# sidd-bme/macaque-3d-pose-estimation

Hardware: AMD Instinct MI355X
Metric: individuals×frames/sec 3D pose (8-view ViTPose-h + triangulate), 1/2/4/8 GPU (higher is better)
Workload: dtype bf16

## Files before the change

### include/mq_hip.h

```cpp
#ifndef MQ_HIP_H
#define MQ_HIP_H

#include <stdint.h>

#ifdef __cplusplus
extern "C" {
#endif

#define MQ_ABI_VERSION 8

typedef struct mq_ctx mq_ctx;
typedef struct mq_vitpose mq_vitpose;

int mq_abi_version(void);
const char* mq_last_error(void);

#define MQ_TUNE_GEMM_FORCE_SMALL 2
#define MQ_TUNE_OPTIM_PCG_ITERS 4
#define MQ_TUNE_GEMM_PINGPONG 12
#define MQ_TUNE_OPTIM_PRECOND_LDS 18
#define MQ_TUNE_GEMM_TILE64 19
#define MQ_TUNE_QKV_HEAD_MAJOR 20
#define MQ_TUNE_OPTIM_STOP 21
#define MQ_TUNE_VIT_RESID_F32 23
#define MQ_TUNE_ATTN_KRING 24
#define MQ_TUNE_OPTIM_TRF_CHUNK 22
#define MQ_TUNE_OPTIM_TRF_FB 25
#define MQ_TUNE_GEMM_W4 27
int mq_set_tuning(int key, int value);
int mq_get_tuning(int key);
int mq_create(int device, mq_ctx** out);
int mq_destroy(mq_ctx* ctx);


int mq_vitpose_create(mq_ctx* ctx, int embed_dims, int num_layers, int num_heads, int ffn_dims, int n_joints,
                      mq_vitpose** out);
int mq_vitpose_destroy(mq_vitpose* model);

int mq_vitpose_set_param(mq_vitpose* model, const char* name, const float* data, int64_t numel, int on_device);

int mq_vitpose_finalize(mq_vitpose* model);

int mq_vitpose_set_graph(mq_vitpose* model, int enable);

int mq_vitpose_timing(mq_vitpose* model, int enable);
int mq_vitpose_timing_result(mq_vitpose* model, double* avg_ms, int* count, int64_t* flops_per_launch);

int mq_crop_udp(mq_ctx* ctx, const uint8_t* frames, int64_t frame_stride, int height, int width,
                const float* boxes, const int32_t* box_frame, int n, float* crops, float* center, float* scale,
                void* stream);

// ... 197 lines not shown
```

### macaque-3d-pose-estimation_amd/csrc/api.cpp

```cpp
#include <hip/hip_runtime.h>

#include <algorithm>
#include <cmath>
#include <cstdio>
#include <cstring>
#include <map>
#include <string>
#include <vector>

#include "bundle.hpp"
#include "cmc.hpp"
#include "geometry.hpp"
#include "overlay.hpp"
#include "detector.hpp"
#include "idcls.hpp"
#include "kernels.hpp"
#include "mq_hip.h"

namespace {

thread_local std::string g_err;
int g_qkv_head_major = 1;
int g_vit_resid_f32 = 0;
int g_tuning_gen = 0;
// ... 127 lines not shown
      break;
    case MQ_TUNE_VIT_RESID_F32:
      g_vit_resid_f32 = value != 0;
      break;
    case MQ_TUNE_ATTN_KRING:
      mq::g_attn_kring = value != 0;
      break;
    case MQ_TUNE_OPTIM_STOP:
      if (value < 0 || value > 7) return fail("mq_set_tuning: optim stop rule must be in [0, 7]", -2);
      mq::g_optim_stop = value;
      break;
    case MQ_TUNE_OPTIM_TRF_CHUNK:
      if (value < 1 || value > 64) return fail("mq_set_tuning: lsmr chunk must be in [1, 64]", -2);
      mq::g_optim_trf_chunk = value;
      break;
    case MQ_TUNE_OPTIM_TRF_FB:
      if (value < 1 || value > 4) return fail("mq_set_tuning: frames per workgroup must be in [1, 4]", -2);
      mq::g_optim_trf_fb = value;
      break;
    case MQ_TUNE_GEMM_W4:
      if (value < 0 || value > 2) return fail("mq_set_tuning: GEMM_W4 must be 0, 1 or 2", -2);
      mq::g_gemm_w4 = value;
      break;
    default:
      return fail("mq_set_tuning: unknown key", -2);
  }
  ++g_tuning_gen;
  return 0;
}

int mq_get_tuning(int key) {
  switch (key) {
    case MQ_TUNE_GEMM_FORCE_SMALL: return mq::g_gemm_force_small ? 1 : 0;
    case MQ_TUNE_GEMM_PINGPONG: return mq::g_gemm_pingpong;
    case MQ_TUNE_OPTIM_PCG_ITERS: return mq::g_optim_pcg_iters;
    case MQ_TUNE_OPTIM_PRECOND_LDS: return mq::g_optim_precond_lds;
    case MQ_TUNE_GEMM_TILE64: return mq::g_gemm_tile64;
    case MQ_TUNE_QKV_HEAD_MAJOR: return g_qkv_head_major;
    case MQ_TUNE_VIT_RESID_F32: return g_vit_resid_f32;
    case MQ_TUNE_ATTN_KRING: return mq::g_attn_kring;
    case MQ_TUNE_OPTIM_STOP: return mq::g_optim_stop;
    case MQ_TUNE_OPTIM_TRF_CHUNK: return mq::g_optim_trf_chunk;
    case MQ_TUNE_OPTIM_TRF_FB: return mq::g_optim_trf_fb;
    case MQ_TUNE_GEMM_W4: return mq::g_gemm_w4;
    default: return fail("mq_get_tuning: unknown key", -2);
  }
}

const char* mq_last_error(void) { return g_err.c_str(); }

int mq_create(int device, mq_ctx** out) {
  if (!out) return fail("mq_create: null out");
  int n = 0;
  HIP_TRY(hipGetDeviceCount(&n));
  if (device < 0 || device >= n) return fail("mq_create: bad device index");
  HIP_TRY(hipSetDevice(device));
  mq_ctx* c = new mq_ctx();
  c->device = device;
  *out = c;
  return 0;
}

int mq_destroy(mq_ctx* ctx) {
  if (!ctx) return 0;
  (void)hipSetDevice(ctx->device);
  ctx->scratch.release();
  ctx->decode_work.release();
// ... 352 lines not shown
      K_TRY(gemm_plain(g, s));
  }
  if (m->L > 0 && !rf32)
    K_TRY(mq::add_layernorm_f32_bf16(m->X, P1, P2, false, m->lnf_g, m->lnf_b, m->Hn, rows, D, 1e-6f, s));
  else
    K_TRY(mq::layernorm_f32_bf16(m->X, m->lnf_g, m->lnf_b, m->Hn, rows, D, 1e-6f, s));
  unsigned short* cols1 = m->G;
  g = mq::GemmArgs{m->Hn, m->w_dc1, cols1, nullptr, nullptr, rows, 16 * dc, D, D, D, 16 * dc, 0};
  K_TRY(gemm_plain(g, s));
  K_TRY(mq::deconv_col2im_bn_relu(cols1, m->bn1_scale, m->bn1_shift, m->Y1, F, m->gh, m->gw, dc, s));
  const int rows2 = F * 4 * T;
  if (m->dc2_subpixel) {
    g = mq::GemmArgs{m->Y1, m->w_dc2, m->Y2, m->bn2_shift4, nullptr, rows2, 4 * dc, 4 * dc, dc, 4 * dc, dc, 0};
    g.conv_h = 2 * m->gh;
    g.conv_w = 2 * m->gw;
    g.conv_c = dc;
    K_TRY(mq::deconv_subpixel_bf16(g, mq::EPI_RELU_BF16, s));
  } else {
    g = mq::GemmArgs{m->Y1, m->w_dc2, m->cols2, nullptr, nullptr, rows2, 16 * dc, dc, dc, dc, 16 * dc, 0};
    K_TRY(mq::gemm_bf16(g, mq::EPI_BF16, s));
    K_TRY(mq::deconv_col2im_bn_relu(m->cols2, m->bn2_scale, m->bn2_shift, m->Y2, F, 2 * m->gh, 2 * m->gw, dc, s));
  }
  const int rows3 = F * 16 * T;
  float* hm_dst = flip ? m->hm_all : heatmaps;
  g = mq::GemmArgs{m->Y2, m->w_fin, hm_dst, m->b_fin, nullptr, rows3, m->J, dc, dc, dc, m->J, 16 * T};
  K_TRY(mq::gemm_bf16(g, mq::EPI_NCHW_F32, s));
  if (flip) K_TRY(mq::flip_average(m->hm_all, heatmaps, n, m->J, 4 * m->gh, 4 * m->gw, m->flip_idx, s));
  return 0;
}

int mq_vitpose_forward(mq_vitpose* m, const float* crops, int n, int flip_test, float* heatmaps, void* stream) {
  if (!m || !crops || !heatmaps) return fail("mq_vitpose_forward: null argument");
  if (!m->finalized) return fail("mq_vitpose_forward: model not finalized", -2);
  if (n <= 0) return 0;
  HIP_TRY(hipSetDevice(m->ctx->device));
  hipStream_t s = (hipStream_t)stream;
  const int F = flip_test ? 2 * n : n;
  int rc = ensure_workspace(m, F);
  if (rc) return rc;
  if (!m->use_graph || m->timing) return launch_forward(m, crops, n, flip_test, heatmaps, s);
  if (!m->cap_stream) {
    HIP_TRY(hipStreamCreateWithFlags(&m->cap_stream, hipStreamNonBlocking));
    HIP_TRY(hipEventCreateWithFlags(&m->ev_in, hipEventDisableTiming));
    HIP_TRY(hipEventCreateWithFlags(&m->ev_out, hipEventDisableTiming));
  }
  hipStream_t cs = m->cap_stream;
// ... 458 lines not shown
  K_TRY(mq::omnidir_undistort(cams, C, pts, out, n, (hipStream_t)stream));
  return 0;
}

int mq_omnidir_project(mq_ctx* ctx, const double* cams, int C, const double* p3d, int n, double* out, void* stream) {
  int rc = check_geo(ctx, cams, C, n);
  if (rc) return rc;
  K_TRY(mq::omnidir_project(cams, C, p3d, out, n, (hipStream_t)stream));
  return 0;
}

int mq_camera_undistort(mq_ctx* ctx, const double* cams, int C, const double* pts, int n, double* out, void* stream) {
  return mq_omnidir_undistort(ctx, cams, C, pts, n, out, stream);
}

int mq_camera_project(mq_ctx* ctx, const double* cams, int C, const double* p3d, int n, double* out, void* stream) {
  return mq_omnidir_project(ctx, cams, C, p3d, n, out, stream);
}

int mq_triangulate_dlt(mq_ctx* ctx, const double* cams, int C, const double* pts, int n, int undistort, double* out,
                       void* stream) {
  int rc = check_geo(ctx, cams, C, n);
  if (rc) return rc;
  if (undistort && n > 0) {
    if (ctx->dlt_ws.ensure((size_t)C * n * 2 * sizeof(double))) return fail("DLT workspace alloc failed", -5);
    K_TRY(mq::omnidir_undistort(cams, C, pts, ctx->dlt_ws.as<double>(), n, (hipStream_t)stream));
    K_TRY(mq::triangulate_dlt(cams, C, ctx->dlt_ws.as<double>(), n, 0, out, (hipStream_t)stream));
    return 0;
  }
  K_TRY(mq::triangulate_dlt(cams, C, pts, n, undistort, out, (hipStream_t)stream));
  return 0;
}

int mq_reproj_error(mq_ctx* ctx, const double* cams, int C, const double* p3d, const double* p2d, int n, int mean,
                    double* out, void* stream) {
  int rc = check_geo(ctx, cams, C, n);
  if (rc) return rc;
  K_TRY(mq::reprojection_error(cams, C, p3d, p2d, n, mean, out, (hipStream_t)stream));
  return 0;
}

int mq_triangulate_ransac(mq_ctx* ctx, const double* cams, int C, const double* pts, int n, int min_cams,
                          double threshold, double* p3d, uint8_t* picked, double* p2d, double* err, void* stream) {
  int rc = check_geo(ctx, cams, C, n);
  if (rc) return rc;
  K_TRY(mq::triangulate_ransac(cams, C, pts, n, min_cams, threshold, p3d, picked, p2d, err, (hipStream_t)stream));
  return 0;
// ... 467 lines not shown
```

### macaque-3d-pose-estimation_amd/csrc/geometry.hip

```cpp
#include "common.hpp"
#include "camera.hpp"
#include "geometry.hpp"
#include "dlt_dev.hpp"

namespace mq {

template <int MAXC>
__device__ __forceinline__ void dlt_point(const double* cams, int C, const double* ux, const double* uy,
                                          unsigned use, double out[3]) {
  double a[4][2 * MAXC];
#pragma unroll
  for (int c = 0; c < MAXC; ++c) {
    const bool on = (c < C) && ((use >> c) & 1u);
    if (on) {
      const CamParams& cp = cam_at(cams, c);
      const double P0[4] = {cp.R[0], cp.R[1], cp.R[2], cp.t[0]};
      const double P1[4] = {cp.R[3], cp.R[4], cp.R[5], cp.t[1]};
      const double P2[4] = {cp.R[6], cp.R[7], cp.R[8], cp.t[2]};
#pragma unroll
      for (int k = 0; k < 4; ++k) {
        a[k][2 * c] = ux[c] * P2[k] - P0[k];
        a[k][2 * c + 1] = uy[c] * P2[k] - P1[k];
      }
    } else {
// ... 193 lines not shown
  unsigned use = 0;
  int cnt = 0;
#pragma unroll
  for (int c = 0; c < MAXC; ++c) {
    ux[c] = 0;
    uy[c] = 0;
    if (c < C) {
      const double u = pts[2 * ((size_t)c * N + n)], v = pts[2 * ((size_t)c * N + n) + 1];
      double x = u, y = v;
      if (undistort) cam_undistort(cam_at(cams, c), u, v, x, y);
      ux[c] = x;
      uy[c] = y;
      if (!(x != x)) {
        use |= 1u << c;
        ++cnt;
      }
    }
  }
  double r[3] = {NAN, NAN, NAN};
  if (cnt >= 2) dlt_point<MAXC>(cams, C, ux, uy, use, r);
  out[3 * n] = r[0];
  out[3 * n + 1] = r[1];
  out[3 * n + 2] = r[2];
}

__global__ void reproj_kernel(const double* __restrict__ cams, int C, const double* __restrict__ p3d,
                              const double* __restrict__ p2d, int N, int mean, double* __restrict__ out) {
  const int n = blockIdx.x * blockDim.x + threadIdx.x;
  if (n >= N) return;
  const double X = p3d[3 * n], Y = p3d[3 * n + 1], Z = p3d[3 * n + 2];
  double sum = 0.0, cnt = 0.0;
  for (int c = 0; c < C; ++c) {
    double u, v;
    cam_project(cam_at(cams, c), X, Y, Z, u, v);
    const size_t o = 2 * ((size_t)c * N + n);
    const double ex = p2d[o] - u, ey = p2d[o + 1] - v;
    if (!mean) {
      out[o] = ex;
      out[o + 1] = ey;
    } else {
      const double nr = sqrt(ex * ex + ey * ey);
      if (!(nr != nr)) {
        sum = sum + nr;
        cnt = cnt + 1.0;
      }
    }
// ... 316 lines not shown
    double* o = out + ((((size_t)a * F + i) * V.C + c) * V.J + j) * 3;
    o[0] = r[0];
    o[1] = r[1];
    o[2] = r[2];
  }
}

int omnidir_undistort(const double* cams, int C, const double* pts, double* out, int N, hipStream_t s) {
  const int tot = C * N;
  if (tot <= 0) return 0;
  hipLaunchKernelGGL(undistort_kernel, dim3((tot + 255) / 256), dim3(256), 0, s, cams, C, pts, out, N);
  return hipGetLastError() == hipSuccess ? 0 : -1;
}

int omnidir_project(const double* cams, int C, const double* p3d, double* out, int N, hipStream_t s) {
  const int tot = C * N;
  if (tot <= 0) return 0;
  hipLaunchKernelGGL(project_kernel, dim3((tot + 255) / 256), dim3(256), 0, s, cams, C, p3d, out, N);
  return hipGetLastError() == hipSuccess ? 0 : -1;
}

int triangulate_dlt(const double* cams, int C, const double* pts, int N, int undistort, double* out, hipStream_t s) {
  if (N <= 0) return 0;
  if (C <= 8)
    hipLaunchKernelGGL(triangulate_kernel<8>, dim3((N + 63) / 64), dim3(64), 0, s, cams, C, pts, N, undistort, out);
  else if (C <= 16)
    hipLaunchKernelGGL(triangulate_kernel<16>, dim3((N + 63) / 64), dim3(64), 0, s, cams, C, pts, N, undistort, out);
  else
    return -2;
  return hipGetLastError() == hipSuccess ? 0 : -1;
}

int reprojection_error(const double* cams, int C, const double* p3d, const double* p2d, int N, int mean, double* out,
                       hipStream_t s) {
  if (N <= 0) return 0;
  hipLaunchKernelGGL(reproj_kernel, dim3((N + 127) / 128), dim3(128), 0, s, cams, C, p3d, p2d, N, mean, out);
  return hipGetLastError() == hipSuccess ? 0 : -1;
}

int triangulate_ransac(const double* cams, int C, const double* pts, int N, int min_cams, double threshold,
                       double* p3d, uint8_t* picked, double* p2d, double* err, hipStream_t s) {
  if (N <= 0) return 0;
  if (C <= 8)
    hipLaunchKernelGGL(ransac_kernel<8>, dim3(N), dim3(64), 0, s, cams, C, pts, N, min_cams, threshold, p3d, picked,
                       p2d, err);
  else if (C <= 16)
// ... 71 lines not shown
```

### macaque-3d-pose-estimation_amd/csrc/geometry.hpp

```cpp
#pragma once
#include <hip/hip_runtime.h>
#include <stdint.h>

namespace mq {
int omnidir_undistort(const double* cams, int C, const double* pts, double* out, int N, hipStream_t s);
int omnidir_project(const double* cams, int C, const double* p3d, double* out, int N, hipStream_t s);
int triangulate_dlt(const double* cams, int C, const double* pts, int N, int undistort, double* out, hipStream_t s);
int reprojection_error(const double* cams, int C, const double* p3d, const double* p2d, int N, int mean, double* out,
                       hipStream_t s);
int triangulate_ransac(const double* cams, int C, const double* pts, int N, int min_cams, double threshold,
                       double* p3d, uint8_t* picked, double* p2d, double* err, hipStream_t s);
int triangulate_pinv(const double* cams, int C, const double* und, const uint8_t* use, int N, double* out,
                     hipStream_t s);
int geometry_affinity(const double* cams, int C, const double* pts, const int32_t* cam_of_det, int B, int M, int J,
                      double thr_kp, double* rays, double* dist, double* out, hipStream_t s);
int viterbi_filter(const double* kp, int A, int F, int C, int J, double score_thr, int n_back, double thres_dist,
                   void* scratch, double* out, hipStream_t s);
size_t viterbi_scratch_bytes(int A, int F, int C, int J, int n_back);
int match_svt(const double* S, const int32_t* n_det, const int32_t* cam_of_det, int B, int Nmax, double alpha,
              double lambda, double mu, double tol, int max_iter, int pselect, void* ws, uint8_t* match,
              double* x_out, int32_t* iters, hipStream_t s);
size_t match_svt_workspace_bytes(int B, int Nmax);
int tracklet_traces(const double* cams, int C, const int32_t* row_start, const int32_t* row_tid,
                    const double* row_kp, int R, int F, int J, const int32_t* trk, int K, const int32_t* cells,
                    int N, double thr_kp, double* p3d, double* median, double* mean, hipStream_t s);
int tracklet_id_votes(int C, const int32_t* row_start, const int32_t* row_tid, const int32_t* row_cls,
                      const double* row_score, int R, int F, const int32_t* trk, int K, const int32_t* cells, int N,
                      double conf_thr, int n_class, int32_t* votes, hipStream_t s);
}
```

### macaque-3d-pose-estimation_amd/csrc/imgproc.hip

```cpp
#include "common.hpp"
#include "kernels.hpp"

namespace mq {

struct BoxWarp {
  float c0, c1, s0, s1;
  double M[6];
};

__device__ __forceinline__ BoxWarp box_warp(const float* bb, int out_w, int out_h) {
  BoxWarp w;
  const float x1 = bb[0], y1 = bb[1], x2 = bb[2], y2 = bb[3];
  const float sw = (x2 - x1) * 1.25f, sh = (y2 - y1) * 1.25f;
  w.c0 = (x2 + x1) * 0.5f;
  w.c1 = (y2 + y1) * 0.5f;
  const float ar = 0.75f;
  if (sw > sh * ar) {
    w.s0 = sw;
    w.s1 = sw / ar;
  } else {
    w.s0 = sh * ar;
    w.s1 = sh;
  }
  const double in0 = (double)(w.c0 * 2.0f), in1 = (double)(w.c1 * 2.0f);
// ... 54 lines not shown
#pragma unroll
  for (int tap = 0; tap < 4; ++tap) {
    const int yy = sy + (tap >> 1), xx = sx + (tap & 1);
    const int wgt = tap == 0 ? w00 : tap == 1 ? w01 : tap == 2 ? w10 : w11;
    if (yy >= 0 && yy < H && xx >= 0 && xx < W) {
      const uint8_t* p = img + ((int64_t)yy * W + xx) * 3;
      acc[0] += p[0] * wgt;
      acc[1] += p[1] * wgt;
      acc[2] += p[2] * wgt;
    }
  }
  const float mean[3] = {123.675f, 116.28f, 103.53f};
  const float stdv[3] = {58.395f, 57.12f, 57.375f};
  const int64_t plane = (int64_t)out_h * out_w;
  float* out = crops + (int64_t)n * 3 * plane + (int64_t)y * out_w + x;
#pragma unroll
  for (int c = 0; c < 3; ++c) {
    int v = (acc[2 - c] + 16384) >> 15;
    v = v < 0 ? 0 : (v > 255 ? 255 : v);
    out[c * plane] = ((float)v - mean[c]) / stdv[c];
  }
}

int crop_udp(const uint8_t* frames, int64_t frame_stride, int img_h, int img_w, const float* boxes,
             const int32_t* box_frame, int n, float* crops, float* center, float* scale, hipStream_t s) {
  if (n <= 0) return 0;
  const int out_w = 192, out_h = 256;
  hipLaunchKernelGGL(crop_udp_kernel, dim3(out_h, n), dim3(256), 0, s, frames, frame_stride, img_h, img_w, boxes,
                     box_frame, crops, center, scale, out_w, out_h);
  return hipGetLastError() == hipSuccess ? 0 : -1;
}

__global__ void flip_average_kernel(const float* __restrict__ hm, float* __restrict__ avg, int N, int K, int HH,
                                    int WW, const int32_t* __restrict__ fi) {
  const int64_t plane = (int64_t)HH * WW;
  const int64_t total = (int64_t)N * K * plane;
  for (int64_t i = blockIdx.x * (int64_t)blockDim.x + threadIdx.x; i < total; i += (int64_t)gridDim.x * blockDim.x) {
    const int x = (int)(i % WW);
    const int y = (int)((i / WW) % HH);
    const int k = (int)((i / plane) % K);
    const int n = (int)(i / (plane * K));
    const float a = hm[i];
    const float b = hm[(((int64_t)(n + N) * K + fi[k]) * HH + y) * WW + (WW - 1 - x)];
    avg[i] = (a + b) * 0.5f;
  }
}

int flip_average(const float* hm_all, float* avg, int n, int joints, int h, int w, const int32_t* flip_idx,
                 hipStream_t s) {
  const int64_t total = (int64_t)n * joints * h * w;
  int blocks = (int)((total + 255) / 256);
  if (blocks > 8192) blocks = 8192;
  hipLaunchKernelGGL(flip_average_kernel, dim3(blocks), dim3(256), 0, s, hm_all, avg, n, joints, h, w, flip_idx);
  return hipGetLastError() == hipSuccess ? 0 : -1;
}

__constant__ float kGauss11[11] = {
    0.00881222914904356f, 0.027143577113747597f, 0.06511405855417252f, 0.12164907157421112f,
    0.17699836194515228f, 0.2005654126405716f,   0.17699836194515228f, 0.12164907157421112f,
    0.06511405855417252f, 0.027143577113747597f, 0.00881222914904356f};

__global__ __launch_bounds__(256) void decode_blur_kernel(const float* __restrict__ avg, int K, int HH, int WW,
                                                          float* __restrict__ work, int32_t* __restrict__ argmax,
                                                          float* __restrict__ score) {
  extern __shared__ __attribute__((aligned(16))) float sm[];
  const int nk = blockIdx.x;
  const int plane = HH * WW;
  const int PR = HH + 10;
  float* hmap = sm;
  float* rows = sm + plane;
  __shared__ float red_v[256];
  __shared__ int red_i[256];
  const float* src = avg + (int64_t)nk * plane;
  float bv = -INFINITY;
  int bi = 0x7fffffff;
  for (int i = threadIdx.x; i < plane; i += blockDim.x) {
// ... 50 lines not shown
  }
  __syncthreads();
  float lmax = -INFINITY;
  for (int i = threadIdx.x; i < plane; i += blockDim.x) {
    const int y = i / WW, x = i % WW;
    float acc = kGauss11[0] * rows[y * WW + x];
    for (int t = 1; t < 11; ++t) acc = acc + kGauss11[t] * rows[(y + t) * WW + x];
    hmap[i] = acc;
    lmax = fmaxf(lmax, acc);
  }
  __syncthreads();
  red_v[threadIdx.x] = lmax;
  __syncthreads();
  for (int o = 128; o > 0; o >>= 1) {
    if (threadIdx.x < o) red_v[threadIdx.x] = fmaxf(red_v[threadIdx.x], red_v[threadIdx.x + o]);
    __syncthreads();
  }
  const float ratio = origin_max / red_v[0];
  float* dst = work + (int64_t)nk * plane;
  for (int i = threadIdx.x; i < plane; i += blockDim.x) {
    float v = hmap[i] * ratio;
    v = fminf(fmaxf(v, 0.001f), 50.0f);
    dst[i] = logf(v);
  }
}

__device__ __forceinline__ float padded_at(const float* work_inst, int K, int HH, int WW, long idx) {
  const long per = (long)(HH + 2) * (WW + 2);
  const long total = per * K;
  if (idx < 0) idx += total;
  const int k = (int)(idx / per);
  const int rem = (int)(idx % per);
  int pr = rem / (WW + 2) - 1, pc = rem % (WW + 2) - 1;
  pr = pr < 0 ? 0 : (pr >= HH ? HH - 1 : pr);
  pc = pc < 0 ? 0 : (pc >= WW ? WW - 1 : pc);
  return work_inst[((long)k * HH + pr) * WW + pc];
}

__global__ void decode_refine_kernel(const float* __restrict__ work, const int32_t* __restrict__ argmax,
                                     const float* __restrict__ score, int N, int K, int HH, int WW,
                                     const float* __restrict__ center, const float* __restrict__ scale, int in_w,
                                     int in_h, double* __restrict__ kp_img, float* __restrict__ kp_hm) {
  const int i = blockIdx.x * blockDim.x + threadIdx.x;
  if (i >= N * K) return;
  const int n = i / K, k = i % K;
  const float* wi = work + (long)n * K * HH * WW;
// ... 36 lines not shown
    b1 = b1 / p;
    inv[0][j] = b1;
    inv[1][j] = b2;
  }
  const double stx = inv[0][0] * (double)dx + inv[0][1] * (double)dy;
  const double sty = inv[1][0] * (double)dx + inv[1][1] * (double)dy;
  const float kx = (float)((double)lx - stx);
  const float ky = (float)((double)ly - sty);
  if (kp_hm) {
    kp_hm[2 * i] = kx;
    kp_hm[2 * i + 1] = ky;
  }
  const double ix = (double)kx / (double)(WW - 1) * (double)in_w;
  const double iy = (double)ky / (double)(HH - 1) * (double)in_h;
  const float s0 = scale[2 * n], s1 = scale[2 * n + 1];
  const float h0 = 0.5f * s0, h1 = 0.5f * s1;
  kp_img[2 * i] = ix / (double)in_w * (double)s0 + (double)center[2 * n] - (double)h0;
  kp_img[2 * i + 1] = iy / (double)in_h * (double)s1 + (double)center[2 * n + 1] - (double)h1;
}

int udp_decode(const float* avg, int n, int joints, int h, int w, const float* center, const float* scale, int in_w,
               int in_h, float* work, double* kp_img, float* score, int32_t* argmax, float* kp_hm, hipStream_t s) {
  if (n <= 0) return 0;
  const size_t lds = (size_t)(h * w + (h + 10) * w) * sizeof(float);
  hipLaunchKernelGGL(decode_blur_kernel, dim3(n * joints), dim3(256), lds, s, avg, joints, h, w, work, argmax, score);
  const int tot = n * joints;
  hipLaunchKernelGGL(decode_refine_kernel, dim3((tot + 127) / 128), dim3(128), 0, s, work, argmax, score, n, joints, h,
                     w, center, scale, in_w, in_h, kp_img, kp_hm);
  return hipGetLastError() == hipSuccess ? 0 : -1;
}

}
```

### macaque-3d-pose-estimation_amd/csrc/kernels.hpp

```cpp
#pragma once
#include <hip/hip_runtime.h>
#include <stdint.h>

namespace mq {

enum GemmEpilogue {
  EPI_BF16 = 0,
  EPI_GELU_BF16 = 1,
  EPI_RESID_F32 = 2,
  EPI_POS_F32 = 3,
  EPI_F32 = 4,
  EPI_NCHW_F32 = 5,
  EPI_RELU_BF16 = 6,
  EPI_RESID_RELU = 7,
};

struct GemmArgs {
  const unsigned short* A;
  const unsigned short* W;
  void* C;
  const float* bias;
  const float* aux;
  int M, N, K;
  int lda, ldw, ldc;
// ... 15 lines not shown
int conv_small_bf16(const GemmArgs& p, int epi, hipStream_t stream);
int deconv_subpixel_bf16(const GemmArgs& p, int epi, hipStream_t stream);
extern bool g_gemm_force_small;
extern int g_gemm_tile64;
extern int g_gemm_pingpong;
bool gemm_pingpong_fits(const GemmArgs& p, int epi, int num_cus);
int gemm_pingpong(const GemmArgs& p, int epi, int num_cus, hipStream_t stream);
int gemm_pingpong_conv(const GemmArgs& p, int epi, int num_cus, hipStream_t stream);
int gemm_pingpong_deconv(const GemmArgs& p, int epi, int num_cus, hipStream_t stream);
extern int g_gemm_w4;
bool gemm_w4_fits(const GemmArgs& p, int epi);
int gemm_w4(const GemmArgs& p, int epi, int num_cus, hipStream_t stream);

int layernorm_f32_bf16(const float* x, const float* gamma, const float* beta, unsigned short* y, int rows, int dim,
                       float eps, hipStream_t s);
int layernorm_f32_f32(const float* x, const float* gamma, const float* beta, float* y, int rows, int dim, float eps,
                      hipStream_t s);
int add_layernorm_f32_bf16(float* x, const unsigned short* p1, const unsigned short* p2, bool store_x,
                           const float* gamma, const float* beta, unsigned short* y, int rows, int dim, float eps,
                           hipStream_t s);
extern int g_attn_kring;
int attention_bf16(const unsigned short* qkv, unsigned short* out, int n_img, int tokens, int dim, int heads,
                   hipStream_t s, bool head_major = false);
int patch_im2col(const float* crops, unsigned short* A, int n_crops, int flip_copies, int img_h, int img_w,
                 int patch, int pad, hipStream_t s);
int deconv_col2im_bn_relu(const unsigned short* cols, const float* scale, const float* shift, unsigned short* out,
                          int n_img, int in_h, int in_w, int ch, hipStream_t s);
int convert_f32_bf16(const float* src, unsigned short* dst, int64_t n, hipStream_t s);
int deconv_weight_pack(const float* w, unsigned short* dst, int cin, int cout, hipStream_t s);
int deconv_subpixel_pack(const float* w, const float* scale, unsigned short* dst, int cin, int cout, hipStream_t s);

int crop_udp(const uint8_t* frames, int64_t frame_stride, int img_h, int img_w, const float* boxes,
             const int32_t* box_frame, int n, float* crops, float* center, float* scale, hipStream_t s);
int flip_average(const float* hm_all, float* avg, int n, int joints, int h, int w, const int32_t* flip_idx,
                 hipStream_t s);
int udp_decode(const float* avg, int n, int joints, int h, int w, const float* center, const float* scale,
               int in_w, int in_h, float* work, double* kp_img, float* score, int32_t* argmax, float* kp_hm,
               hipStream_t s);

extern int g_optim_pcg_iters;
extern int g_optim_stop;
extern int g_optim_precond_lds;
size_t optim_workspace_bytes(int B, int F, int J, int NL);
int optim_points(const double* cams, int C, const double* p2d, double* x, int B, int F, int J, const int* cons_host,
                 int n_strong, int n_weak, const double* ssf_host, double scale_length, double scale_length_weak,
                 double rp, int loss, int n_deriv, int fix_lengths, int max_iter, double ftol, void* ws,
                 double* stats, hipStream_t s);
extern int g_optim_trf_chunk;
extern int g_optim_trf_fb;
size_t optim_trf_workspace_bytes(int B, int F, int J, int C, int NL);
int optim_points_trf(const double* cams, int C, const double* p2d, double* x, int B, int F, int J, const int* cons_host,
                     int n_strong, int n_weak, const double* ssf_host, double scale_length, double scale_length_weak,
                     double rp, int loss, int n_deriv, int fix_lengths, int max_nfev, double ftol, void* ws,
                     double* stats, hipStream_t s);

}
```

### macaque-3d-pose-estimation_amd/csrc/vit_ops.hip

```cpp
#include "common.hpp"
#include "kernels.hpp"

namespace mq {

template <int MAXIT, bool OUT_F32, int NADD, bool STORE_X>
__global__ __launch_bounds__(256) void layernorm_kernel(float* __restrict__ x, const bf16_t* __restrict__ p1,
                                                         const bf16_t* __restrict__ p2, const float* __restrict__ g,
                                                         const float* __restrict__ b, void* __restrict__ yv,
                                                         int rows, int dim, float eps) {
  const int lane = threadIdx.x & 63;
  const int row = blockIdx.x * 4 + (threadIdx.x >> 6);
  if (row >= rows) return;
  float* xr = x + (size_t)row * dim;
  float4 v[MAXIT], gg[MAXIT], bb[MAXIT];
  uint2 pa[MAXIT], pb[MAXIT];
#pragma unroll
  for (int it = 0; it < MAXIT; ++it) {
    const int i = it * 256 + lane * 4;
    pa[it] = pb[it] = make_uint2(0u, 0u);
    if (i < dim) {
      v[it] = *reinterpret_cast<const float4*>(xr + i);
      if constexpr (NADD >= 1) pa[it] = *reinterpret_cast<const uint2*>(p1 + (size_t)row * dim + i);
      if constexpr (NADD >= 2) pb[it] = *reinterpret_cast<const uint2*>(p2 + (size_t)row * dim + i);
      gg[it] = *reinterpret_cast<const float4*>(g + i);
// ... 467 lines not shown
    const int src = f % n;
    const bool flip = f >= n;
    const int py = t / gw, px = t % gw;
    const int k0 = kc * 8;
    const int ci = k0 / (P * P);
    const int ky = (k0 / P) % P;
    const int kx0 = k0 % P;
    const int y = py * P + ky - pad;
    const float* plane = crops + ((int64_t)src * 3 + ci) * IH * IW;
    float v[8];
#pragma unroll
    for (int e = 0; e < 8; ++e) {
      int x = px * P + kx0 + e - pad;
      bool ok = (y >= 0) && (y < IH) && (x >= 0) && (x < IW);
      int xs = flip ? (IW - 1 - x) : x;
      v[e] = ok ? plane[(int64_t)y * IW + xs] : 0.f;
    }
    uint4 o = make_uint4(pack_bf16x2(v[0], v[1]), pack_bf16x2(v[2], v[3]), pack_bf16x2(v[4], v[5]),
                         pack_bf16x2(v[6], v[7]));
    *reinterpret_cast<uint4*>(A + m * K + k0) = o;
  }
}

int patch_im2col(const float* crops, unsigned short* A, int n_crops, int flip_copies, int img_h, int img_w, int patch,
                 int pad, hipStream_t s) {
  if ((patch * patch) % 8) return -1;
  const int gh = (img_h + 2 * pad - patch) / patch + 1;
  const int gw = (img_w + 2 * pad - patch) / patch + 1;
  const int64_t total = (int64_t)n_crops * flip_copies * gh * gw * (3 * patch * patch / 8);
  int blocks = (int)((total + 255) / 256);
  if (blocks > 8192) blocks = 8192;
  hipLaunchKernelGGL(patch_im2col_kernel, dim3(blocks), dim3(256), 0, s, crops, A, n_crops, flip_copies, img_h, img_w,
                     patch, pad, gh, gw);
  return hipGetLastError() == hipSuccess ? 0 : -2;
}

__global__ void col2im_bn_relu_kernel(const bf16_t* __restrict__ cols, const float* __restrict__ scale,
                                      const float* __restrict__ shift, bf16_t* __restrict__ out, int n, int IH,
                                      int IW, int C) {
  const int OH = IH * 2, OW = IW * 2;
  const int c8 = C / 8;
  const int64_t total = (int64_t)n * OH * OW * c8;
  for (int64_t idx = blockIdx.x * (int64_t)blockDim.x + threadIdx.x; idx < total;
       idx += (int64_t)gridDim.x * blockDim.x) {
    const int cc = (int)(idx % c8);
    const int64_t pix = idx / c8;
    const int ox = (int)(pix % OW);
    const int oy = (int)((pix / OW) % OH);
    const int img = (int)(pix / ((int64_t)OW * OH));
    float acc[8];
#pragma unroll
// ... 102 lines not shown
```

Measured before the change: 250.8.

## Add fused flip head, row-based im2col/crop, strip decode blur, wave-parallel DLT

Adds several new kernels, all enabled by default. A fused final-conv head does both the normal and flipped 1x1 GEMMs with MFMA and averages them in one pass, removing the hm_all buffer and the flip_average kernel. The patch im2col and UDP crop move to row-oriented kernels with vectorized loads. A specialized 64x48 decode blur uses static LDS and strip convolution. DLT triangulation fuses undistortion into a per-point wave kernel using DPP reductions and Jacobi SVD, which may change numerical behaviour compared with the previous path.

```diff
diff --git a/include/mq_hip.h b/include/mq_hip.h
--- a/include/mq_hip.h
+++ b/include/mq_hip.h
@@ -27,6 +27,11 @@
 #define MQ_TUNE_OPTIM_TRF_CHUNK 22
 #define MQ_TUNE_OPTIM_TRF_FB 25
 #define MQ_TUNE_GEMM_W4 27
+#define MQ_TUNE_HEAD_FUSED 29
+#define MQ_TUNE_DLT_VIEWS 30
+#define MQ_TUNE_IM2COL_ROWS 31
+#define MQ_TUNE_DECODE_STRIPS 32
+#define MQ_TUNE_CROP_ROWS 33
 int mq_set_tuning(int key, int value);
 int mq_get_tuning(int key);
 int mq_create(int device, mq_ctx** out);
diff --git a/macaque-3d-pose-estimation_amd/csrc/api.cpp b/macaque-3d-pose-estimation_amd/csrc/api.cpp
--- a/macaque-3d-pose-estimation_amd/csrc/api.cpp
+++ b/macaque-3d-pose-estimation_amd/csrc/api.cpp
@@ -173,6 +173,22 @@
       if (value < 0 || value > 2) return fail("mq_set_tuning: GEMM_W4 must be 0, 1 or 2", -2);
       mq::g_gemm_w4 = value;
       break;
+    case MQ_TUNE_HEAD_FUSED:
+      mq::g_head_fused = value != 0;
+      break;
+    case MQ_TUNE_DLT_VIEWS:
+      if (value < 0 || value > 2) return fail("mq_set_tuning: DLT_VIEWS must be 0, 1 or 2", -2);
+      mq::g_dlt_views = value;
+      break;
+    case MQ_TUNE_IM2COL_ROWS:
+      mq::g_im2col_rows = value != 0;
+      break;
+    case MQ_TUNE_DECODE_STRIPS:
+      mq::g_decode_strips = value != 0;
+      break;
+    case MQ_TUNE_CROP_ROWS:
+      mq::g_crop_rows = value != 0;
+      break;
     default:
       return fail("mq_set_tuning: unknown key", -2);
   }
@@ -194,6 +210,11 @@
     case MQ_TUNE_OPTIM_TRF_CHUNK: return mq::g_optim_trf_chunk;
     case MQ_TUNE_OPTIM_TRF_FB: return mq::g_optim_trf_fb;
     case MQ_TUNE_GEMM_W4: return mq::g_gemm_w4;
+    case MQ_TUNE_HEAD_FUSED: return mq::g_head_fused;
+    case MQ_TUNE_DLT_VIEWS: return mq::g_dlt_views;
+    case MQ_TUNE_IM2COL_ROWS: return mq::g_im2col_rows;
+    case MQ_TUNE_DECODE_STRIPS: return mq::g_decode_strips;
+    case MQ_TUNE_CROP_ROWS: return mq::g_crop_rows;
     default: return fail("mq_get_tuning: unknown key", -2);
   }
 }
@@ -592,6 +613,10 @@
     K_TRY(mq::deconv_col2im_bn_relu(m->cols2, m->bn2_scale, m->bn2_shift, m->Y2, F, 2 * m->gh, 2 * m->gw, dc, s));
   }
   const int rows3 = F * 16 * T;
+  if (flip && mq::head_flip_fits(heatmaps, m->J, 4 * m->gh, 4 * m->gw, dc)) {
+    K_TRY(mq::head_flip(m->Y2, m->w_fin, m->b_fin, m->flip_idx, heatmaps, n, m->J, 4 * m->gh, 4 * m->gw, s));
+    return 0;
+  }
   float* hm_dst = flip ? m->hm_all : heatmaps;
   g = mq::GemmArgs{m->Y2, m->w_fin, hm_dst, m->b_fin, nullptr, rows3, m->J, dc, dc, dc, m->J, 16 * T};
   K_TRY(mq::gemm_bf16(g, mq::EPI_NCHW_F32, s));
@@ -1096,7 +1121,7 @@
                        void* stream) {
   int rc = check_geo(ctx, cams, C, n);
   if (rc) return rc;
-  if (undistort && n > 0) {
+  if (undistort && n > 0 && !mq::g_dlt_views) {
     if (ctx->dlt_ws.ensure((size_t)C * n * 2 * sizeof(double))) return fail("DLT workspace alloc failed", -5);
     K_TRY(mq::omnidir_undistort(cams, C, pts, ctx->dlt_ws.as<double>(), n, (hipStream_t)stream));
     K_TRY(mq::triangulate_dlt(cams, C, ctx->dlt_ws.as<double>(), n, 0, out, (hipStream_t)stream));
diff --git a/macaque-3d-pose-estimation_amd/csrc/geometry.hip b/macaque-3d-pose-estimation_amd/csrc/geometry.hip
--- a/macaque-3d-pose-estimation_amd/csrc/geometry.hip
+++ b/macaque-3d-pose-estimation_amd/csrc/geometry.hip
@@ -239,6 +239,135 @@
   out[3 * n] = r[0];
   out[3 * n + 1] = r[1];
   out[3 * n + 2] = r[2];
+}
+
+int g_dlt_views = 2;
+
+template <int MAXC>
+__global__ __launch_bounds__(64) void triangulate_views_kernel(const double* __restrict__ cams, int C,
+                                                               const double* __restrict__ pts, int N,
+                                                               double* __restrict__ out) {
+  constexpr int PPW = 64 / MAXC;
+  const int lane = threadIdx.x;
+  const int c = lane % MAXC;
+  const int n = blockIdx.x * PPW + lane / MAXC;
+  double x = 0, y = 0;
+  if (c < C && n < N) {
+    const double u = pts[2 * ((size_t)c * N + n)], v = pts[2 * ((size_t)c * N + n) + 1];
+    cam_undistort(cam_at(cams, c), u, v, x, y);
+  }
+  double ux[MAXC], uy[MAXC];
+  unsigned use = 0;
+  int cnt = 0;
+#pragma unroll
+  for (int k = 0; k < MAXC; ++k) {
+    ux[k] = __shfl(x, lane - c + k, 64);
+    uy[k] = __shfl(y, lane - c + k, 64);
+    if (k < C && !(ux[k] != ux[k])) {
+      use |= 1u << k;
+      ++cnt;
+    }
+  }
+  if (c != 0 || n >= N) return;
+  double r[3] = {NAN, NAN, NAN};
+  if (cnt >= 2) dlt_point<MAXC>(cams, C, ux, uy, use, r);
+  out[3 * n] = r[0];
+  out[3 * n + 1] = r[1];
+  out[3 * n + 2] = r[2];
+}
+
+template <int CTRL>
+__device__ __forceinline__ double dpp_row_add(double v) {
+  const int lo = __builtin_amdgcn_update_dpp(0, __double2loint(v), CTRL, 0xF, 0xF, false);
+  const int hi = __builtin_amdgcn_update_dpp(0, __double2hiint(v), CTRL, 0xF, 0xF, false);
+  return v + __hiloint2double(hi, lo);
+}
+__device__ __forceinline__ double row16_sum(double v) {
+  v = dpp_row_add<0xB1>(v);
+  v = dpp_row_add<0x4E>(v);
+  v = dpp_row_add<0x141>(v);
+  return dpp_row_add<0x140>(v);
+}
+
+__global__ __launch_bounds__(64) void triangulate_rows_kernel(const double* __restrict__ cams, int C,
+                                                              const double* __restrict__ pts, int N,
+                                                              double* __restrict__ out) {
+  const int lane = threadIdx.x;
+  const int r = lane & 15, c = r >> 1;
+  const int n = blockIdx.x * 4 + (lane >> 4);
+  const bool live = n < N;
+  double x = NAN, y = NAN;
+  if (live && c < C) {
+    const double u = pts[2 * ((size_t)c * N + n)], v = pts[2 * ((size_t)c * N + n) + 1];
+    cam_undistort(cam_at(cams, c), u, v, x, y);
+  }
+  const bool on = live && c < C && !(x != x);
+  const unsigned rowbits = (unsigned)(__ballot(on) >> (lane & 48)) & 0xffffu;
+  const bool run = live && __popc(rowbits) >= 4;
+  double a[4] = {0.0, 0.0, 0.0, 0.0};
+  if (on) {
+    const CamParams& cp = cam_at(cams, c);
+    const double P2[4] = {cp.R[6], cp.R[7], cp.R[8], cp.t[2]};
+    const double uv = (r & 1) ? y : x;
+#pragma unroll
+    for (int k = 0; k < 4; ++k) a[k] = uv * P2[k] - ((r & 1) ? (k < 3 ? cp.R[3 + k] : cp.t[1]) : (k < 3 ? cp.R[k] : cp.t[0]));
+  }
+  double res[3] = {NAN, NAN, NAN};
+  if (run) {
+    double V[4][4];
+#pragma unroll
+    for (int i = 0; i < 4; ++i)
+#pragma unroll
+      for (int j = 0; j < 4; ++j) V[i][j] = (i == j) ? 1.0 : 0.0;
+    for (int sweep = 0; sweep < 30; ++sweep) {
+      bool rotated = false;
+#pragma unroll
+      for (int p = 0; p < 3; ++p) {
+#pragma unroll
+        for (int q = p + 1; q < 4; ++q) {
+          const double alpha = row16_sum(a[p] * a[p]);
+          const double beta = row16_sum(a[q] * a[q]);
+          const double gamma = row16_sum(a[p] * a[q]);
+          if (fabs(gamma) > 1e-15 * sqrt(alpha * beta) && gamma != 0.0) {
+            rotated = true;
+            const double zeta = (beta - alpha) / (2.0 * gamma);
+            const double t = (zeta >= 0 ? 1.0 : -1.0) / (fabs(zeta) + sqrt(1.0 + zeta * zeta));
+            const double cs = 1.0 / sqrt(1.0 + t * t);
+            const double sn = cs * t;
+            const double ap = a[p], aq = a[q];
+            a[p] = cs * ap - sn * aq;
+            a[q] = sn * ap + cs * aq;
+#pragma unroll
+            for (int i = 0; i < 4; ++i) {
+              const double vp = V[p][i], vq = V[q][i];
+              V[p][i] = cs * vp - sn * vq;
+              V[q][i] = sn * vp + cs * vq;
+            }
+          }
+        }
+      }
+      if (!rotated) break;
+    }
+    double sig[4];
+#pragma unroll
+    for (int j = 0; j < 4; ++j) sig[j] = sqrt(row16_sum(a[j] * a[j]));
+    double smin = sig[0], v[4] = {V[0][0], V[0][1], V[0][2], V[0][3]};
+#pragma unroll
+    for (int j = 1; j < 4; ++j)
+      if (sig[j] < smin) {
+        smin = sig[j];
+#pragma unroll
+        for (int k = 0; k < 4; ++k) v[k] = V[j][k];
+      }
+    res[0] = v[0] / v[3];
+    res[1] = v[1] / v[3];
+    res[2] = v[2] / v[3];
+  }
+  if (live && r == 0) {
+    out[3 * n] = res[0];
+    out[3 * n + 1] = res[1];
+    out[3 * n + 2] = res[2];
+  }
 }
 
 __global__ void reproj_kernel(const double* __restrict__ cams, int C, const double* __restrict__ p3d,
@@ -601,6 +730,15 @@
 
 int triangulate_dlt(const double* cams, int C, const double* pts, int N, int undistort, double* out, hipStream_t s) {
   if (N <= 0) return 0;
+  if (undistort && g_dlt_views && C <= 16) {
+    if (C <= 8 && g_dlt_views == 2)
+      hipLaunchKernelGGL(triangulate_rows_kernel, dim3((N + 3) / 4), dim3(64), 0, s, cams, C, pts, N, out);
+    else if (C <= 8)
+      hipLaunchKernelGGL(triangulate_views_kernel<8>, dim3((N + 7) / 8), dim3(64), 0, s, cams, C, pts, N, out);
+    else
+      hipLaunchKernelGGL(triangulate_views_kernel<16>, dim3((N + 3) / 4), dim3(64), 0, s, cams, C, pts, N, out);
+    return hipGetLastError() == hipSuccess ? 0 : -1;
+  }
   if (C <= 8)
     hipLaunchKernelGGL(triangulate_kernel<8>, dim3((N + 63) / 64), dim3(64), 0, s, cams, C, pts, N, undistort, out);
   else if (C <= 16)
diff --git a/macaque-3d-pose-estimation_amd/csrc/geometry.hpp b/macaque-3d-pose-estimation_amd/csrc/geometry.hpp
--- a/macaque-3d-pose-estimation_amd/csrc/geometry.hpp
+++ b/macaque-3d-pose-estimation_amd/csrc/geometry.hpp
@@ -6,6 +6,7 @@
 int omnidir_undistort(const double* cams, int C, const double* pts, double* out, int N, hipStream_t s);
 int omnidir_project(const double* cams, int C, const double* p3d, double* out, int N, hipStream_t s);
 int triangulate_dlt(const double* cams, int C, const double* pts, int N, int undistort, double* out, hipStream_t s);
+extern int g_dlt_views;
 int reprojection_error(const double* cams, int C, const double* p3d, const double* p2d, int N, int mean, double* out,
                        hipStream_t s);
 int triangulate_ransac(const double* cams, int C, const double* pts, int N, int min_cams, double threshold,
diff --git a/macaque-3d-pose-estimation_amd/csrc/imgproc.hip b/macaque-3d-pose-estimation_amd/csrc/imgproc.hip
--- a/macaque-3d-pose-estimation_amd/csrc/imgproc.hip
+++ b/macaque-3d-pose-estimation_amd/csrc/imgproc.hip
@@ -100,12 +100,77 @@
   }
 }
 
+int g_crop_rows = 1;
+
+template <int ROWS>
+__global__ __launch_bounds__(192) void crop_udp_rows_kernel(const uint8_t* __restrict__ frames, int64_t fstride, int H,
+                                                            int W, const float* __restrict__ boxes,
+                                                            const int32_t* __restrict__ box_frame,
+                                                            float* __restrict__ crops, float* __restrict__ center,
+                                                            float* __restrict__ scale, int out_w, int out_h) {
+  const int y0 = blockIdx.x * ROWS;
+  const int n = blockIdx.y;
+  const int x = threadIdx.x;
+  const BoxWarp bw = box_warp(boxes + 4 * n, out_w, out_h);
+  if (y0 == 0 && x == 0) {
+    center[2 * n] = bw.c0;
+    center[2 * n + 1] = bw.c1;
+    scale[2 * n] = bw.s0;
+    scale[2 * n + 1] = bw.s1;
+  }
+  if (x >= out_w) return;
+  const int ad = __double2int_rn(bw.M[0] * (double)x * 1024.0);
+  const int bd = __double2int_rn(bw.M[3] * (double)x * 1024.0);
+  const uint8_t* img = frames + (int64_t)box_frame[n] * fstride;
+  const float mean[3] = {123.675f, 116.28f, 103.53f};
+  const float stdv[3] = {58.395f, 57.12f, 57.375f};
+  const int64_t plane = (int64_t)out_h * out_w;
+#pragma unroll
+  for (int dy = 0; dy < ROWS; ++dy) {
+    const int y = y0 + dy;
+    if (y >= out_h) break;
+    const int X0 = __double2int_rn((bw.M[1] * (double)y + bw.M[2]) * 1024.0) + 16;
+    const int Y0 = __double2int_rn((bw.M[4] * (double)y + bw.M[5]) * 1024.0) + 16;
+    const int X = (X0 + ad) >> 5;
+    const int Y = (Y0 + bd) >> 5;
+    const int sx = X >> 5, sy = Y >> 5;
+    const int fx = X & 31, fy = Y & 31;
+    const int w00 = (32 - fy) * (32 - fx) * 32, w01 = (32 - fy) * fx * 32;
+    const int w10 = fy * (32 - fx) * 32, w11 = fy * fx * 32;
+    int acc[3] = {0, 0, 0};
+#pragma unroll
+    for (int tap = 0; tap < 4; ++tap) {
+      const int yy = sy + (tap >> 1), xx = sx + (tap & 1);
+      const int wgt = tap == 0 ? w00 : tap == 1 ? w01 : tap == 2 ? w10 : w11;
+      if (yy >= 0 && yy < H && xx >= 0 && xx < W) {
+        const uint8_t* p = img + ((int64_t)yy * W + xx) * 3;
+        acc[0] += p[0] * wgt;
+        acc[1] += p[1] * wgt;
+        acc[2] += p[2] * wgt;
+      }
+    }
+    float* out = crops + (int64_t)n * 3 * plane + (int64_t)y * out_w + x;
+#pragma unroll
+    for (int c = 0; c < 3; ++c) {
+      int v = (acc[2 - c] + 16384) >> 15;
+      v = v < 0 ? 0 : (v > 255 ? 255 : v);
+      out[c * plane] = ((float)v - mean[c]) / stdv[c];
+    }
+  }
+}
+
 int crop_udp(const uint8_t* frames, int64_t frame_stride, int img_h, int img_w, const float* boxes,
              const int32_t* box_frame, int n, float* crops, float* center, float* scale, hipStream_t s) {
   if (n <= 0) return 0;
   const int out_w = 192, out_h = 256;
-  hipLaunchKernelGGL(crop_udp_kernel, dim3(out_h, n), dim3(256), 0, s, frames, frame_stride, img_h, img_w, boxes,
-                     box_frame, crops, center, scale, out_w, out_h);
+  if (g_crop_rows) {
+    constexpr int ROWS = 4;
+    hipLaunchKernelGGL(crop_udp_rows_kernel<ROWS>, dim3((out_h + ROWS - 1) / ROWS, n), dim3(192), 0, s, frames,
+                       frame_stride, img_h, img_w, boxes, box_frame, crops, center, scale, out_w, out_h);
+  } else {
+    hipLaunchKernelGGL(crop_udp_kernel, dim3(out_h, n), dim3(256), 0, s, frames, frame_stride, img_h, img_w, boxes,
+                       box_frame, crops, center, scale, out_w, out_h);
+  }
   return hipGetLastError() == hipSuccess ? 0 : -1;
 }
 
@@ -130,6 +195,93 @@
   int blocks = (int)((total + 255) / 256);
   if (blocks > 8192) blocks = 8192;
   hipLaunchKernelGGL(flip_average_kernel, dim3(blocks), dim3(256), 0, s, hm_all, avg, n, joints, h, w, flip_idx);
+  return hipGetLastError() == hipSuccess ? 0 : -1;
+}
+
+int g_head_fused = 1;
+
+constexpr int HF_K = 256;
+constexpr int HF_PITCH = HF_K * 2 + 16;
+constexpr int HF_GPW = 2;
+
+__global__ __launch_bounds__(256) void head_flip_kernel(const bf16_t* __restrict__ Y2, const bf16_t* __restrict__ W,
+                                                        const float* __restrict__ bias,
+                                                        const int32_t* __restrict__ fi, float* __restrict__ out,
+                                                        int n, int J, int HW, int WW, int groups) {
+  __shared__ __attribute__((aligned(16))) char wl[2 * 32 * HF_PITCH];
+  for (int c = threadIdx.x; c < 2 * 32 * (HF_K / 8); c += 256) {
+    const int chunk = c & (HF_K / 8 - 1), row = (c / (HF_K / 8)) & 31, set = c / (32 * (HF_K / 8));
+    int src = row < J ? row : J - 1;
+    if (set) src = fi[src];
+    *reinterpret_cast<uint4*>(wl + (set * 32 + row) * HF_PITCH + chunk * 16) =
+        *reinterpret_cast<const uint4*>(W + (size_t)src * HF_K + chunk * 8);
+  }
+  __syncthreads();
+  const int lane = threadIdx.x & 63, wave = threadIdx.x >> 6;
+  const int r = lane & 15, fk = lane >> 4;
+  float ba[2], bb[2];
+#pragma unroll
+  for (int j = 0; j < 2; ++j) {
+    const int ch = r + 16 * j < J ? r + 16 * j : J - 1;
+    ba[j] = bias[ch];
+    bb[j] = bias[fi[ch]];
+  }
+#pragma unroll 1
+  for (int t = 0; t < HF_GPW; ++t) {
+    const int g = (blockIdx.x * HF_GPW + t) * 4 + wave;
+    if (g >= groups) break;
+    const int p0 = g * 16;
+    const int img = p0 / HW, pix = p0 - img * HW;
+    const int y = pix / WW, x0 = pix - y * WW;
+    const bf16_t* ra = Y2 + ((size_t)img * HW + pix + r) * HF_K + fk * 8;
+    const bf16_t* rb = Y2 + ((size_t)(img + n) * HW + y * WW + (WW - 1 - (x0 + r))) * HF_K + fk * 8;
+    bf16x8 a[HF_K / 32], b[HF_K / 32];
+#pragma unroll
+    for (int kk = 0; kk < HF_K / 32; ++kk) {
+      a[kk] = *reinterpret_cast<const bf16x8*>(ra + kk * 32);
+      b[kk] = *reinterpret_cast<const bf16x8*>(rb + kk * 32);
+    }
+    f32x4 ca[2], cb[2];
+#pragma unroll
+    for (int j = 0; j < 2; ++j) ca[j] = cb[j] = f32x4{0.f, 0.f, 0.f, 0.f};
+#pragma unroll
+    for (int kk = 0; kk < HF_K / 32; ++kk) {
+#pragma unroll
+      for (int j = 0; j < 2; ++j) {
+        const char* w0 = wl + (j * 16 + r) * HF_PITCH + (kk * 4 + fk) * 16;
+        const bf16x8 wa = *reinterpret_cast<const bf16x8*>(w0);
+        const bf16x8 wb = *reinterpret_cast<const bf16x8*>(w0 + 32 * HF_PITCH);
+        ca[j] = __builtin_amdgcn_mfma_f32_16x16x32_bf16(a[kk], wa, ca[j], 0, 0, 0);
+        cb[j] = __builtin_amdgcn_mfma_f32_16x16x32_bf16(b[kk], wb, cb[j], 0, 0, 0);
+      }
+    }
+#pragma unroll
+    for (int j = 0; j < 2; ++j) {
+      const int ch = r + 16 * j;
+      if (ch >= J) continue;
+      float4 o;
+      o.x = ((ca[j][0] + ba[j]) + (cb[j][0] + bb[j])) * 0.5f;
+      o.y = ((ca[j][1] + ba[j]) + (cb[j][1] + bb[j])) * 0.5f;
+      o.z = ((ca[j][2] + ba[j]) + (cb[j][2] + bb[j])) * 0.5f;
+      o.w = ((ca[j][3] + ba[j]) + (cb[j][3] + bb[j])) * 0.5f;
+      *reinterpret_cast<float4*>(out + ((size_t)img * J + ch) * HW + pix + fk * 4) = o;
+    }
+  }
+}
+
+bool head_flip_fits(const float* heatmaps, int joints, int h, int w, int channels) {
+  return g_head_fused && channels == HF_K && joints >= 1 && joints <= 32 && h > 0 && w > 0 && w % 16 == 0 &&
+         (reinterpret_cast<uintptr_t>(heatmaps) & 15) == 0;
+}
+
+int head_flip(const unsigned short* y2, const unsigned short* w, const float* bias, const int32_t* flip_idx,
+              float* heatmaps, int n, int joints, int h, int wd, hipStream_t s) {
+  if (n <= 0) return 0;
+  if ((int64_t)n * h * wd >= (1ll << 31)) return -1;
+  const int groups = n * h * wd / 16;
+  const int per_block = 4 * HF_GPW;
+  hipLaunchKernelGGL(head_flip_kernel, dim3((groups + per_block - 1) / per_block), dim3(256), 0, s, y2, w, bias,
+                     flip_idx, heatmaps, n, joints, h * wd, wd, groups);
   return hipGetLastError() == hipSuccess ? 0 : -1;
 }
 
@@ -226,6 +378,130 @@
     float v = hmap[i] * ratio;
     v = fminf(fmaxf(v, 0.001f), 50.0f);
     dst[i] = logf(v);
+  }
+}
+
+int g_decode_strips = 1;
+
+constexpr int DB_H = 64, DB_W = 48;
+constexpr int DB_PP = DB_W + 11;
+constexpr int DB_RP = DB_W + 1;
+
+__device__ __forceinline__ bool blur_takes(float v2, int i2, float v1, int i1) {
+  const bool n1 = v1 != v1, n2 = v2 != v2;
+  if (n1 || n2) return n2 && (!n1 || i2 < i1);
+  return (v2 > v1) || (v2 == v1 && i2 < i1);
+}
+
+__global__ __launch_bounds__(256) void decode_blur64x48_kernel(const float* __restrict__ avg,
+                                                               float* __restrict__ work,
+                                                               int32_t* __restrict__ argmax,
+                                                               float* __restrict__ score) {
+  __shared__ float P[DB_H * DB_PP];
+  __shared__ float R[(DB_H + 10) * DB_RP];
+  __shared__ float red_v[4];
+  __shared__ int red_i[4];
+  __shared__ float red_m[4];
+  const int nk = blockIdx.x;
+  const int tid = threadIdx.x;
+  const int lane = tid & 63, wave = tid >> 6;
+  constexpr int plane = DB_H * DB_W;
+  const float* src = avg + (int64_t)nk * plane;
+  float bv = -INFINITY;
+  int bi = 0x7fffffff;
+#pragma unroll
+  for (int q = 0; q < plane / 4 / 256; ++q) {
+    const int i4 = tid + 256 * q;
+    const float4 v4 = *reinterpret_cast<const float4*>(src + 4 * i4);
+    const int y = (4 * i4) / DB_W, x = (4 * i4) % DB_W;
+    const float v[4] = {v4.x, v4.y, v4.z, v4.w};
+#pragma unroll
+    for (int e = 0; e < 4; ++e) {
+      P[y * DB_PP + 5 + x + e] = v[e];
+      const int i = 4 * i4 + e;
+      if (v[e] > bv || (v[e] == bv && i < bi) || (v[e] != v[e] && bv == bv)) {
+        bv = v[e];
+        bi = i;
+      }
+    }
+  }
+  for (int i = tid; i < DB_H * 11; i += 256) {
+    const int y = i / 11, c = i % 11;
+    P[y * DB_PP + (c < 5 ? c : DB_W + c)] = 0.f;
+  }
+  for (int i = tid; i < 10 * DB_RP; i += 256) {
+    const int r = i / DB_RP, c = i % DB_RP;
+    R[((r < 5 ? r : DB_H + r)) * DB_RP + c] = 0.f;
+  }
+#pragma unroll
+  for (int o = 32; o > 0; o >>= 1) {
+    const float v2 = __shfl_xor(bv, o, 64);
+    const int i2 = __shfl_xor(bi, o, 64);
+    if (blur_takes(v2, i2, bv, bi)) {
+      bv = v2;
+      bi = i2;
+    }
+  }
+  if (lane == 0) {
+    red_v[wave] = bv;
+    red_i[wave] = bi;
+  }
+  __syncthreads();
+  float origin_max = red_v[0];
+  int origin_i = red_i[0];
+#pragma unroll
+  for (int w = 1; w < 4; ++w)
+    if (blur_takes(red_v[w], red_i[w], origin_max, origin_i)) {
+      origin_max = red_v[w];
+      origin_i = red_i[w];
+    }
+  if (tid == 0) {
+    argmax[nk] = origin_i;
+    score[nk] = origin_max;
+  }
+  {
+    const int y = tid & 63, x0 = (tid >> 6) * 12;
+    float in[22];
+#pragma unroll
+    for (int j = 0; j < 22; ++j) in[j] = P[y * DB_PP + x0 + j];
+#pragma unroll
+    for (int j = 0; j < 12; ++j) {
+      float acc = kGauss11[0] * in[j];
+#pragma unroll
+      for (int t = 1; t < 11; ++t) acc = acc + kGauss11[t] * in[j + t];
+      R[(y + 5) * DB_RP + x0 + j] = acc;
+    }
+  }
+  __syncthreads();
+  float bl[16];
+  float lmax = -INFINITY;
+  const int cx = tid % DB_W, cy0 = (tid / DB_W) * 16;
+  const bool col = tid < DB_W * (DB_H / 16);
+  if (col) {
+    float in[26];
+#pragma unroll
+    for (int j = 0; j < 26; ++j) in[j] = R[(cy0 + j) * DB_RP + cx];
+#pragma unroll
+    for (int j = 0; j < 16; ++j) {
+      float acc = kGauss11[0] * in[j];
+#pragma unroll
+      for (int t = 1; t < 11; ++t) acc = acc + kGauss11[t] * in[j + t];
+      bl[j] = acc;
+      lmax = fmaxf(lmax, acc);
+    }
+  }
+  lmax = wave_max(lmax);
+  if (lane == 0) red_m[wave] = lmax;
+  __syncthreads();
+  const float ratio = origin_max / fmaxf(fmaxf(red_m[0], red_m[1]), fmaxf(red_m[2], red_m[3]));
+  if (col) {
+    float* dst = work + (int64_t)nk * plane + cy0 * DB_W + cx;
+#pragma unroll
+    for (int j = 0; j < 16; ++j) {
+      float v = bl[j] * ratio;
+      v = fminf(fmaxf(v, 0.001f), 50.0f);
+      dst[j * DB_W] = logf(v);
+    }
   }
 }
 
@@ -308,8 +584,13 @@
 int udp_decode(const float* avg, int n, int joints, int h, int w, const float* center, const float* scale, int in_w,
                int in_h, float* work, double* kp_img, float* score, int32_t* argmax, float* kp_hm, hipStream_t s) {
   if (n <= 0) return 0;
-  const size_t lds = (size_t)(h * w + (h + 10) * w) * sizeof(float);
-  hipLaunchKernelGGL(decode_blur_kernel, dim3(n * joints), dim3(256), lds, s, avg, joints, h, w, work, argmax, score);
+  if (g_decode_strips && h == DB_H && w == DB_W && (reinterpret_cast<uintptr_t>(avg) & 15) == 0) {
+    hipLaunchKernelGGL(decode_blur64x48_kernel, dim3(n * joints), dim3(256), 0, s, avg, work, argmax, score);
+  } else {
+    const size_t lds = (size_t)(h * w + (h + 10) * w) * sizeof(float);
+    hipLaunchKernelGGL(decode_blur_kernel, dim3(n * joints), dim3(256), lds, s, avg, joints, h, w, work, argmax,
+                       score);
+  }
   const int tot = n * joints;
   hipLaunchKernelGGL(decode_refine_kernel, dim3((tot + 127) / 128), dim3(128), 0, s, work, argmax, score, n, joints, h,
                      w, center, scale, in_w, in_h, kp_img, kp_hm);
diff --git a/macaque-3d-pose-estimation_amd/csrc/kernels.hpp b/macaque-3d-pose-estimation_amd/csrc/kernels.hpp
--- a/macaque-3d-pose-estimation_amd/csrc/kernels.hpp
+++ b/macaque-3d-pose-estimation_amd/csrc/kernels.hpp
@@ -61,6 +61,7 @@
 extern int g_attn_kring;
 int attention_bf16(const unsigned short* qkv, unsigned short* out, int n_img, int tokens, int dim, int heads,
                    hipStream_t s, bool head_major = false);
+extern int g_im2col_rows;
 int patch_im2col(const float* crops, unsigned short* A, int n_crops, int flip_copies, int img_h, int img_w,
                  int patch, int pad, hipStream_t s);
 int deconv_col2im_bn_relu(const unsigned short* cols, const float* scale, const float* shift, unsigned short* out,
@@ -73,6 +74,12 @@
              const int32_t* box_frame, int n, float* crops, float* center, float* scale, hipStream_t s);
 int flip_average(const float* hm_all, float* avg, int n, int joints, int h, int w, const int32_t* flip_idx,
                  hipStream_t s);
+extern int g_crop_rows;
+extern int g_decode_strips;
+extern int g_head_fused;
+bool head_flip_fits(const float* heatmaps, int joints, int h, int w, int channels);
+int head_flip(const unsigned short* y2, const unsigned short* w, const float* bias, const int32_t* flip_idx,
+              float* heatmaps, int n, int joints, int h, int wd, hipStream_t s);
 int udp_decode(const float* avg, int n, int joints, int h, int w, const float* center, const float* scale,
                int in_w, int in_h, float* work, double* kp_img, float* score, int32_t* argmax, float* kp_hm,
                hipStream_t s);
diff --git a/macaque-3d-pose-estimation_amd/csrc/vit_ops.hip b/macaque-3d-pose-estimation_amd/csrc/vit_ops.hip
--- a/macaque-3d-pose-estimation_amd/csrc/vit_ops.hip
+++ b/macaque-3d-pose-estimation_amd/csrc/vit_ops.hip
@@ -513,11 +513,58 @@
   }
 }
 
+int g_im2col_rows = 1;
+
+__global__ __launch_bounds__(256) void patch_im2col_rows_kernel(const float* __restrict__ crops,
+                                                                bf16_t* __restrict__ A, int n, int IH, int IW, int P,
+                                                                int pad, int gh, int gw) {
+  const int K = 3 * P * P;
+  const int k8 = K / 8;
+  const int f = blockIdx.x / gh, py = blockIdx.x - f * gh;
+  const int src = f % n;
+  const bool flip = f >= n;
+  const float* img = crops + (size_t)src * 3 * IH * IW;
+  bf16_t* rows = A + ((size_t)f * gh * gw + (size_t)py * gw) * K;
+  for (int i = threadIdx.x; i < gw * k8; i += 256) {
+    const int px = i / k8, kc = i - px * k8;
+    const int k0 = kc * 8;
+    const int ci = k0 / (P * P);
+    const int rem = k0 - ci * P * P;
+    const int ky = rem / P, kx0 = rem - ky * P;
+    const int y = py * P + ky - pad;
+    const int xb = px * P + kx0 - pad;
+    const bool yok = y >= 0 && y < IH;
+    const float* line = img + ((size_t)ci * IH + (yok ? y : 0)) * IW;
+    unsigned o[4];
+#pragma unroll
+    for (int e = 0; e < 4; ++e) {
+      const int x = xb + 2 * e;
+      float2 v = make_float2(0.f, 0.f);
+      if (yok && x >= 0 && x < IW) {
+        if (flip) {
+          const float2 m = *reinterpret_cast<const float2*>(line + (IW - 2 - x));
+          v = make_float2(m.y, m.x);
+        } else {
+          v = *reinterpret_cast<const float2*>(line + x);
+        }
+      }
+      o[e] = pack_bf16x2(v.x, v.y);
+    }
+    *reinterpret_cast<uint4*>(rows + (size_t)px * K + k0) = make_uint4(o[0], o[1], o[2], o[3]);
+  }
+}
+
 int patch_im2col(const float* crops, unsigned short* A, int n_crops, int flip_copies, int img_h, int img_w, int patch,
                  int pad, hipStream_t s) {
   if ((patch * patch) % 8) return -1;
   const int gh = (img_h + 2 * pad - patch) / patch + 1;
   const int gw = (img_w + 2 * pad - patch) / patch + 1;
+  if (g_im2col_rows && patch % 8 == 0 && pad % 2 == 0 && img_w % 2 == 0 &&
+      (reinterpret_cast<uintptr_t>(crops) & 7) == 0 && (int64_t)n_crops * flip_copies * gh < (1ll << 31)) {
+    hipLaunchKernelGGL(patch_im2col_rows_kernel, dim3(n_crops * flip_copies * gh), dim3(256), 0, s, crops, A, n_crops,
+                       img_h, img_w, patch, pad, gh, gw);
+    return hipGetLastError() == hipSuccess ? 0 : -2;
+  }
   const int64_t total = (int64_t)n_crops * flip_copies * gh * gw * (3 * patch * patch / 8);
   int blocks = (int)((total + 255) / 256);
   if (blocks > 8192) blocks = 8192;
```

After: 252.2 (median of 6 runs). No clear change (+0.6%).
